# ecpoppenheimer/TensorFlowRayTrace

Measured on AMD Instinct MI355X. Metric: ray-surface intersection tests/sec (fwd+bwd), higher is better.
Workload: dtype f32 ray state, f32 filter + f64 decisions

## Files before the change

### tensorflowraytrace_amd/csrc/tfrt_trace3d.hip

```cpp
#include <vector>

#include <type_traits>
#include "tfrt_common.h"
#include "goal_finish.h"
#include "wave_schedule.h"

namespace tfrt {

constexpr int TILE = 512;
constexpr int KC = 24;

constexpr int ERR_CAPACITY = 1;


__global__ __launch_bounds__(BLOCK) void k_center(const double* __restrict__ fverts, int M,
                                                  double* __restrict__ c0, int32_t* nrays0, int n,
                                                  int32_t* tail8, unsigned int* scan_ticket) {
  if (nrays0 != nullptr) {
    if (threadIdx.x == 0) *nrays0 = n;
    if (threadIdx.x < 8) tail8[threadIdx.x] = 0;
    if (threadIdx.x == 0 && scan_ticket != nullptr) *scan_ticket = 0u;
  }
  __shared__ double red[WAVES][3];
  __shared__ double ctr[3];
// ... 1303 lines not shown
  return __int_as_float(__builtin_amdgcn_readfirstlane(__float_as_int(v)));
}
__device__ __forceinline__ float bcast_f(float v, int src_lane) {
  return __int_as_float(__builtin_amdgcn_readlane(__float_as_int(v), src_lane));
}

template <typename U>
using LdsPtr = __attribute__((address_space(3))) U*;

template <typename RT>
__device__ __forceinline__ void beam_decide(const int nb, const int lane, LdsPtr<const uint32_t> x_pair,
                                         LdsPtr<const RT> rt, LdsPtr<unsigned long long> best_k,
                                         LdsPtr<int32_t> best_i, const double* __restrict__ fverts,
                                         const double eps_int, const double eps_size,
                                         const double eps_start) {
  bool have = false;
  unsigned long long key = 0, old = 0;
  int j = -1;
  const uint32_t xp = lane < nb ? x_pair[lane] : 0u;
  const int slot = (int)(xp & 63u);
  if (lane < nb) {
    double s[3], e[3];
#pragma unroll
    for (int k = 0; k < 3; ++k) {
      s[k] = static_cast<double>(rt[k * 64 + slot]);
      e[k] = static_cast<double>(rt[(3 + k) * 64 + slot]);
    }
    j = (int)(xp >> 6);
    old = best_k[slot];
    double P[9];
    const double* fp = fverts + 9 * (int64_t)j;
#pragma unroll
    for (int k = 0; k < 9; ++k) P[k] = fp[k];
    const TriHit h = exact_triangle<true>(s, e, P, eps_int, eps_size, eps_start);
    if (h.valid) {
      have = true;
      key = dkey(h.ray_u);
    }
  }
  wave_fence();
  if (have) atomicMin((unsigned long long*)&best_k[slot], key);
  wave_fence();
  bool win = false;
  if (have) {
    const unsigned long long now = best_k[slot];
    win = key == now;
    if (win && now < old) best_i[slot] = 0x7FFFFFFF;
  }
  wave_fence();
  if (win) atomicMin((int32_t*)&best_i[slot], j);
  wave_fence();
}

template <typename RT>
struct BeamLds {
  uint16_t slist[BEAM_SLIST];
  uint16_t clist[BEAM_CLIST];
  uint32_t flist[BEAM_FLIST];
  uint32_t x_pair[192];
  float4 ftab[65][4];
  RT rtab[6][64];
  unsigned long long best_k[64];
  int32_t best_i[64];
};

struct BeamScene {
  const float4* susphere;
  const float4* clsphere;
  const float4* csphere;
  const float4* crec;
  const double* fverts;
  const double* c0;
  int n_clusters, n_super;
  double eps_int, eps_size, eps_start;
};

#ifdef TFRT_TICKS
#define TFRT_WI_ARG _wi
#else
#define TFRT_WI_ARG nullptr
#endif

struct BeamCentre {
  double c[3];
  float cf[3];
};
__device__ __forceinline__ BeamCentre beam_centre(const double* __restrict__ c0) {
  BeamCentre o;
#pragma unroll
  for (int k = 0; k < 3; ++k) {
    o.c[k] = c0[k];
    o.cf[k] = uniform_f((float)o.c[k]);
  }
  return o;
}

template <typename T, typename RT>
__device__ __forceinline__ bool beam_pass(BeamLds<RT>& W, const BeamScene& g,
                                          const BeamCentre& ctr, const int lane,
                                          const int bundle, const bool live, const int skip,
                                          const bool first_pass, const int coherent_only,
                                          unsigned* _wi, unsigned* work = nullptr) {
  TFRT_TICK_INIT;
  const float4* __restrict__ susphere = g.susphere;
  const float4* __restrict__ clsphere = g.clsphere;
  const float4* __restrict__ csphere = g.csphere;
  const float4* __restrict__ crec = g.crec;
  const double* __restrict__ fverts = g.fverts;
  const int n_clusters = g.n_clusters, n_super = g.n_super;
  const double eps_int = g.eps_int, eps_size = g.eps_size, eps_start = g.eps_start;
  const float4 never = make_float4(0.f, 0.f, 0.f, -1.f);
  W.best_k[lane] = dkey(INFINITY);
  W.best_i[lane] = -1;
  const double cx = ctr.c[0], cy = ctr.c[1], cz = ctr.c[2];
  const float cxf = ctr.cf[0], cyf = ctr.cf[1], czf = ctr.cf[2];
  auto rel = [](const RT v, const double c, const float cf) -> float {
    if constexpr (sizeof(T) <= 4) return (float)v - cf;
    else return (float)((double)v - c);
  };
  const float es_f = (float)eps_size;
  int xn = 0;

  auto decide = [&](const int nb) {
    TFRT_STAT(28, 1);
    TFRT_WAVE_NOTE(1, 1);
    wave_fence();
    beam_decide<RT>(nb, lane, (LdsPtr<const uint32_t>)&W.x_pair[0],
                    (LdsPtr<const RT>)&W.rtab[0][0], (LdsPtr<unsigned long long>)&W.best_k[0],
                    (LdsPtr<int32_t>)&W.best_i[0], fverts, eps_int, eps_size, eps_start);
  };

  TFRT_STAT(8, 1);
  constexpr int BEAM_ATTEMPTS = 20;
  TFRT_TICK(0);
  float gap = -1.f;
  unsigned long long cuts = 0ull;
  int lo = 0, attempts = 0;
  bool spread = false;
  while (lo < bundle) {
    ++attempts;
    TFRT_STAT(30, 1);
    TFRT_WAVE_NOTE(0, 1);
    const unsigned long long above = lo < 63 ? (cuts >> (lo + 1)) << (lo + 1) : 0ull;
    const int hi = above != 0ull ? __ffsll((long long)above) - 1 : bundle;
    const int len = hi - lo;
    wave_fence();
    RT own[6];
#pragma unroll
    for (int k = 0; k < 6; ++k) own[k] = W.rtab[k][lane];
    const float sx = rel(own[0], cx, cxf), sy = rel(own[1], cy, cyf), sz = rel(own[2], cz, czf);
    const float dx = (float)(own[3] - own[0]), dy = (float)(own[4] - own[1]),
                dz = (float)(own[5] - own[2]);
    const float len2 = dx * dx + dy * dy + dz * dz;
    const bool ok = live && len2 > 0.f && len2 < 3.0e38f;
    const float inv = ok ? __builtin_amdgcn_rsqf(len2) : 0.f;
    const float ux = dx * inv, uy = dy * inv, uz = dz * inv;
    const float rabs = fabsf(sx) + fabsf(sy) + fabsf(sz);
    const bool sel = ok && lane >= lo && lane < hi;
    const float4 su_first = lane < n_super ? susphere[lane] : never;
    const float cnt = (float)__popcll(__ballot(sel));
    bool narrow = true, brute = false;
    int ns = 0, nc = 0, nf = 0;
    Beam bm = {0.f, 0.f, 0.f, 0.f, 0.f, 1.f, 0.f, 0.f, -INFINITY, 1.f, 0.f, 0.f, 0.f, 1.f, 0.f,
               INFINITY, 0.f};
    float ray_t = 0.f, ray_dt = 0.f, ray_terr = 0.f;
    float Ax = 0.f, Ay = 0.f, Mx = 0.f, My = 0.f, Mlen = 0.f, Perr = 0.f, Pm = 0.f;
    if (cnt > 0.f) {
      float swx = sel ? ux : 0.f, swy = sel ? uy : 0.f, swz = sel ? uz : 0.f;
      float sox = sel ? sx : 0.f, soy = sel ? sy : 0.f, soz = sel ? sz : 0.f;
      float Lw = sel ? rabs : 0.f;
      wave_sum4(swx, swy, swz, sox);
      wave_sum2_max(soy, soz, Lw);
      const float wl2 = swx * swx + swy * swy + swz * swz;
      narrow = wl2 > 0.49f * cnt * cnt;
      spread = !narrow;
      const float wi = narrow ? __builtin_amdgcn_rsqf(wl2) : 0.f;
      bm.wx = swx * wi; bm.wy = swy * wi; bm.wz = swz * wi;
      const float icnt = __builtin_amdgcn_rcpf(cnt);
      bm.ox = sox * icnt; bm.oy = soy * icnt; bm.oz = soz * icnt;
      const float cosk = ux * bm.wx + uy * bm.wy + uz * bm.wz;
      if (__any(sel && !(cosk > 0.7f))) narrow = false, spread = true;
      const float px = sx - bm.ox, py = sy - bm.oy, pz = sz - bm.oz;
      const float ts = px * bm.wx + py * bm.wy + pz * bm.wz;
      ray_t = ts;
      ray_dt = dx * bm.wx + dy * bm.wy + dz * bm.wz;
      ray_terr = 1e-5f * (rabs + fabsf(bm.ox) + fabsf(bm.oy) + fabsf(bm.oz));
      {
        const float f0 = fabsf(bm.wx), f1 = fabsf(bm.wy), f2 = fabsf(bm.wz);
        const bool k0 = f0 <= f1 && f0 <= f2, k1 = !k0 && f1 <= f2;
        const float kx = k0 ? 1.f : 0.f, ky = k1 ? 1.f : 0.f, kz = (!k0 && !k1) ? 1.f : 0.f;
        const float cxx = bm.wy * kz - bm.wz * ky, cyy = bm.wz * kx - bm.wx * kz,
                    czz = bm.wx * ky - bm.wy * kx;
// ... 60 lines not shown
      }
      wave_fence();
      TFRT_TICK(2);
      if (narrow && ns > 0) {
        for (int b = 0; b < ns * SUPER; b += 64) {
          const int k = b + lane;
          bool hit = false;
          int cl = 0;
          if (k < ns * SUPER) {
            cl = (int)W.slist[k >> 3] * SUPER + (k & 7);
            if (cl < n_clusters) hit = beam_touch(bm, clsphere[cl]);
          }
          const unsigned long long m = __ballot(hit);
          if (hit) {
            const int pos = nc + rank_below(m);
            if (pos < BEAM_CLIST) W.clist[pos] = (uint16_t)cl;
          }
          nc += __popcll(m);
        }
        narrow = nc <= BEAM_CLIST && n_clusters <= 65536;
      }
      wave_fence();
      TFRT_TICK(3);
      if (narrow && nc > 0) {
        for (int b = 0; b < nc * CLUSTER; b += 64) {
          const int k = b + lane;
          bool hit = false;
          unsigned slot = 0;
          if (k < nc * CLUSTER) {
            slot = (unsigned)W.clist[k >> 4] * CLUSTER + (unsigned)(k & 15);
            hit = beam_touch(bm, csphere[slot]);
          }
          const unsigned long long m = __ballot(hit);
          if (hit) {
            const int pos = nf + rank_below(m);
            if (pos < BEAM_FLIST) W.flist[pos] = slot;
          }
          nf += __popcll(m);
        }
        narrow = nf <= BEAM_FLIST && !(nf > BEAM_WIDE && len > 8 && attempts <= 6);
      }
      wave_fence();
      TFRT_TICK(4);
    }
    if (!narrow) {
      TFRT_TICK(10);
      const bool hopeless = !coherent_only &&
                            ((len == bundle && (spread || (nc > 64 && nc > n_clusters / 4))) ||
                             attempts >= BEAM_ATTEMPTS);
      if (len > 1 && !hopeless) {
        if (cuts == 0ull) {
          const float su = sx * ux + sy * uy + sz * uz;
          const float fx = sx - su * ux, fy = sy - su * uy, fz = sz - su * uz;
          const float gx = fx - __shfl_up(fx, 1, 64), gy = fy - __shfl_up(fy, 1, 64),
                      gz = fz - __shfl_up(fz, 1, 64);
          const float hx = ux - __shfl_up(ux, 1, 64), hy = uy - __shfl_up(uy, 1, 64),
                      hz = uz - __shfl_up(uz, 1, 64);
          const bool prev_ok = __shfl_up(ok ? 1 : 0, 1, 64) != 0;
          gap = 0.f;
          if (ok && prev_ok && lane > 0)
            gap = gx * gx + gy * gy + gz * gz +
                  (sx * sx + sy * sy + sz * sz) * (hx * hx + hy * hy + hz * hz);
          if (!(gap >= 0.f)) gap = 0.f;
        }
        const bool inside = lane > lo && lane < hi;
        const float widest = wave_max_f(inside ? gap : -1.f);
        const unsigned long long at = __ballot(inside && gap == widest);
        const int g = (widest > 0.f && at != 0ull) ? __ffsll((long long)at) - 1 : lo + (len >> 1);
        cuts |= 1ull << g;
        continue;
      }
      if (len == 1 && !hopeless) {
        brute = true;
      } else {
        TFRT_STAT(ns > BEAM_SLIST ? 10 : (nc > BEAM_CLIST ? 11 : (nf > BEAM_FLIST ? 12 : 9)), 1);
        TFRT_STAT(15, lo);
        return false;
      }
    }

    TFRT_STAT(13, nf);
    TFRT_WAVE_NOTE(3, nf);
    TFRT_TICK(5);
    auto reach_now = [&]() {
      const double best = dkey_inv(W.best_k[lane]);
      const float bu = next_up_f((float)best) * ray_dt;
      return ray_t + bu + 1e-5f * fabsf(bu) + ray_terr;
    };
    float myreach = reach_now();
    bool queued = false;
    const int n_cand = brute ? n_clusters * CLUSTER : nf;
    int f0 = 0;
    do {
      const int nb = min(64, n_cand - f0);
      if (work != nullptr) work[1] += (unsigned)nb;
      float4 rec[4] = {never, never, never, never};
      bool touch = false;
      float tnear = INFINITY;
      bool cand = lane < nb;
      if (brute && cand) {
        const float4 sp = csphere[f0 + lane];
        const float vx = sp.x - bm.ox, vy = sp.y - bm.oy, vz = sp.z - bm.oz;
        const float vu = vx * bm.wx + vy * bm.wy + vz * bm.wz;
        const float v2 = vx * vx + vy * vy + vz * vz;
        const float rr = __builtin_amdgcn_sqrtf(sp.w) * 1.000002f + bm.radius(vu, 0.f);
        cand = v2 - vu * vu <= rr * rr + 4e-6f * v2;
      }
      if (cand) {
        const int64_t memb = brute ? (int64_t)(f0 + lane) : (int64_t)W.flist[f0 + lane];
        const float4 r0 = crec[3 * memb], r1 = crec[3 * memb + 1], r2 = crec[3 * memb + 2];
        touch = face_frame(bm, r0, r1, r2, es_f, rec) && __float_as_int(r0.w) >= 0;
        tnear = rec[0].w;
        if (tnear != tnear) tnear = -INFINITY;
        rec[0].w = tnear;
      }
      f0 += 64;
      const bool closing = f0 >= n_cand && hi == bundle;
      const unsigned long long tm = __ballot(touch);
      const int nt = __popcll(tm);
      int place = 0;
      for (unsigned long long rest = tm; rest != 0ull; rest &= rest - 1ull) {
        const int o = __ffsll((long long)rest) - 1;
        const float to = bcast_f(tnear, o);
        place += (to < tnear || (to == tnear && o < lane)) ? 1 : 0;
      }
      wave_fence();
      if (touch) {
        W.ftab[place][0] = rec[0];
        W.ftab[place][1] = rec[1];
        W.ftab[place][2] = rec[2];
        W.ftab[place][3] = rec[3];
      }
      wave_fence();
      TFRT_STAT(27, nt);
      TFRT_TICK(6);
      float span = -INFINITY;
      auto on_face = [&](const float word, int* j, float* thi) {
        const float tn = bcast_f(word, 3);
        *thi = bcast_f(word, 7);
        *j = __float_as_int(bcast_f(word, 14));
        float room, e0, e1, e2;
        face_edges(word, Ax, Ay, Mx, My, Mlen, Perr, Pm, room, e0, e1, e2);
        const bool behind = bm.tmin > -INFINITY && *thi < ray_t - ray_terr;
        return (sel & (*j != skip) & !(myreach < tn) & !behind) &
               (!(e0 > room) & !(e1 > room) & !(e2 > room));
      };
      for (int c = 0;; c += 2) {
        const bool end = c >= nt;
        const bool two = c + 1 < nt;
        const float* recs = reinterpret_cast<const float*>(&W.ftab[end ? 0 : c][0]) + (lane & 15);
        const float word = recs[0], word2 = recs[16];
        const float tn = end ? INFINITY : bcast_f(word, 3);
        const bool flush =
            end ? closing
                : (tn > span && __ballot(sel && !(queued || myreach < INFINITY)) == 0ull);
        while (xn >= 64 || (flush && xn > 0)) {
          const int nd = min(xn, 64);
          wave_fence();
          decide(nd);
          uint32_t tp = 0u, tq = 0u;
          if (lane < xn - nd) tp = W.x_pair[nd + lane];
          if (lane + 64 < xn - nd) tq = W.x_pair[nd + 64 + lane];
          wave_fence();
          if (lane < xn - nd) W.x_pair[lane] = tp;
          if (lane + 64 < xn - nd) W.x_pair[64 + lane] = tq;
          xn -= nd;
          wave_fence();
          if (xn == 0) queued = false;
          myreach = reach_now();
// ... 327 lines not shown
      const double* fp = fnorm + 3 * (int64_t)tri;
#pragma unroll
      for (int q = 0; q < 3; ++q) un[q] = fp[q];
      if (feta != nullptr) {
        const double* fe = feta + 4 * (int64_t)tri;
        n1 = fe[0];
        n2 = fe[1];
        n_in = fe[2];
      } else {
        double n_out;
        face_indices(sc, tri, rid, &n_in, &n_out);
        snell_ratios(n_in, n_out, &n1, &n2);
      }
      const Snell3 f = snell3d_core(s, h, un, n1, n2, n_in == 0.0);
      rec_cls[i] = (uint8_t)(cls | (f.nu > 0.0 ? TAPE_INTERNAL : 0) | (f.reflect ? TAPE_REFLECT : 0));
      double e2[3];
      for (int k = 0; k < 3; ++k) e2[k] = advance(h[k], L, f.w[k]);
      store_ray3(rays_out, stride_out, slot, h, e2);
      ray_id_out[slot] = rid;
      last_tri_out[slot] = tri;
      rec_slot[i] = slot;
      if (prep_next != nullptr) {
        double sr[3], er[3], u[3], scv[3];
        for (int k = 0; k < 3; ++k) {
          sr[k] = static_cast<double>(static_cast<T>(h[k]));
          er[k] = static_cast<double>(static_cast<T>(e2[k]));
        }
        float o[8];
        ray_filter_state(sr, er, c0, o, u, scv);
#pragma unroll
        for (int k = 0; k < 8; ++k) prep_next[k * pstride + slot] = o[k];
      }
    }
  }
  if (!ok) atomicOr(err, ERR_CAPACITY);
}

inline int inplace_bundle(int64_t N) { return N <= 160 * 1024 ? 32 : 64; }
inline size_t inplace_wstride(int64_t N) { return ((size_t)((N > 0 ? N : 1) + 31) / 32 + 63) / 64 * 64; }

template <typename T>
struct InplaceArgs {
  const T* src;
  int64_t src_stride;
  int32_t N, P, bundle, nwaves;
  const InplaceTape* tape;
  const int32_t* sched;
  int32_t ngroups, gshift;
};

#ifndef TFRT_INPLACE_WAVES
#define TFRT_INPLACE_WAVES 5
#endif
#define TFRT_INPLACE_ATTR __attribute__((amdgpu_waves_per_eu(TFRT_INPLACE_WAVES, TFRT_INPLACE_WAVES)))
template <typename T, bool ROWS>
__device__ __forceinline__ void trace_inplace(const InplaceArgs<T>& a, const BeamScene& g) {
  using RT = std::conditional_t<sizeof(T) <= 4, float, double>;
  const int lane = threadIdx.x;
  int qwave = blockIdx.x;
  if (a.sched != nullptr) {
    const int g = __builtin_amdgcn_readfirstlane(a.sched[blockIdx.x >> a.gshift]);
    if ((unsigned)g >= (unsigned)a.ngroups) return;
    qwave = (g << a.gshift) + ((int)blockIdx.x & ((1 << a.gshift) - 1));
    if (qwave >= a.nwaves) return;
  }
  const int q = qwave * a.bundle + lane;
  const bool has = lane < a.bundle && q < a.N;
  const int64_t i = has ? q : 0;
  __shared__ BeamLds<RT> lds;
  BeamLds<RT>& W = lds;
#pragma unroll
  for (int k = 0; k < 6; ++k) W.rtab[k][lane] = static_cast<RT>(a.src[k * a.src_stride + i]);
  bool active = has;
  int skip = -1;
  int p = 0;
  static_assert(sizeof(InplaceTape) % 4 == 0 && sizeof(InplaceTape) / 4 <= 64, "one word per lane");
  const uint32_t tape_words =
      reinterpret_cast<const uint32_t*>(a.tape)[lane < (int)(sizeof(InplaceTape) / 4) ? lane : 0];
  TFRT_WAVE_BEGIN;
  unsigned work[2] = {0u, 0u};
  const BeamCentre centre = beam_centre(g.c0);
  for (; p < a.P; ++p) {
    if (__ballot(active) == 0ull) break;
    beam_pass<T, RT>(W, g, centre, lane, a.bundle, active, skip, p == 0, 1,
                     TFRT_WI_ARG, work);
    wave_fence();
    TFRT_TICK_INIT;
    uint32_t tw = tape_words;
    __asm__ volatile("" : "+v"(tw));
    InplaceTape tq;
    {
      uint32_t w[sizeof(InplaceTape) / 4];
#pragma unroll
      for (int k = 0; k < (int)(sizeof(InplaceTape) / 4); ++k)
        w[k] = (uint32_t)__builtin_amdgcn_readlane((int)tw, k);
      __builtin_memcpy(&tq, w, sizeof(InplaceTape));
    }
    int cls = -1;
    if (active) {
      const int bi = W.best_i[lane];
      const double t = dkey_inv(W.best_k[lane]);
      int cat = 0;
      double un[3] = {0.0, 0.0, 0.0}, fe[3] = {0.0, 0.0, 0.0};
      if (bi >= 0) {
        cat = tq.catagory[bi];
        const double* fp = tq.fnorm + 3 * (int64_t)bi;
#pragma unroll
        for (int k = 0; k < 3; ++k) un[k] = fp[k];
        if (tq.feta != nullptr) {
          const double* fq = tq.feta + 4 * (int64_t)bi;
#pragma unroll
          for (int k = 0; k < 3; ++k) fe[k] = fq[k];
        }
      }
      cls = (bi < 0) ? CLS_DEAD : cat_to_cls(cat);
      const size_t at = (size_t)p * tq.n + i;
      tq.rec_tri[at] = bi;
      tq.rec_t[at] = t;
      int tape = cls;
      if (cls == CLS_ACTIVE) {
        double s[3], e[3], h[3];
#pragma unroll
        for (int k = 0; k < 3; ++k) {
          s[k] = static_cast<double>(W.rtab[k][lane]);
          e[k] = static_cast<double>(W.rtab[3 + k][lane]);
        }
        hit_point(s, e, t, h);
        double n1, n2, n_in;
        if (tq.feta != nullptr) {
          n1 = fe[0];
          n2 = fe[1];
          n_in = fe[2];
        } else {
          n_in = tq.n_table[(int64_t)tq.mat_in[bi] * tq.n_table_stride + i];
          const double n_out = tq.n_table[(int64_t)tq.mat_out[bi] * tq.n_table_stride + i];
          snell_ratios(n_in, n_out, &n1, &n2);
        }
        const Snell3 f = snell3d_core(s, h, un, n1, n2, n_in == 0.0);
        tape |= (f.nu > 0.0 ? TAPE_INTERNAL : 0) | (f.reflect ? TAPE_REFLECT : 0);
        T* out = static_cast<T*>(tq.rays_ws) + (size_t)p * 6 * tq.n;
#pragma unroll
        for (int k = 0; k < 3; ++k) {
          const T hs = static_cast<T>(h[k]);
          const T es = static_cast<T>(advance(h[k], tq.L, f.w[k]));
          out[k * tq.n + i] = hs;
          out[(3 + k) * tq.n + i] = es;
          W.rtab[k][lane] = static_cast<RT>(hs);
          W.rtab[3 + k][lane] = static_cast<RT>(es);
        }
        skip = bi;
      } else {
        active = false;
        if (ROWS) {
          const bool fin = cls == CLS_FINISHED;
          T* fin_rows = static_cast<T*>(tq.fin_rows);
          double h[3] = {0.0, 0.0, 0.0};
          if (fin) {
            double s[3], e[3];
#pragma unroll
            for (int k = 0; k < 3; ++k) {
              s[k] = static_cast<double>(W.rtab[k][lane]);
              e[k] = static_cast<double>(W.rtab[3 + k][lane]);
            }
            hit_point(s, e, t, h);
          }
#pragma unroll
          for (int k = 0; k < 3; ++k) {
            fin_rows[k * tq.fin_cap + i] = fin ? static_cast<T>(W.rtab[k][lane]) : a.src[k * a.src_stride + i];
            fin_rows[(3 + k) * tq.fin_cap + i] = fin ? static_cast<T>(h[k]) : a.src[(3 + k) * a.src_stride + i];
          }
          tq.fin_face[i] = fin ? bi : -1;
          tq.fin_passes[i] = p + 1;
        }
      }
      tq.rec_cls[at] = (uint8_t)tape;
    }
    uint32_t word = 0u;
#pragma unroll
    for (int c = 0; c < 4; ++c) word |= (uint32_t)__popcll(__ballot(cls == c)) << (8 * c);
    if (lane == 0) tq.wcount[(size_t)p * tq.wstride + qwave] = word;
    TFRT_TICK(11);
  }
  InplaceTape te;
  {
    uint32_t w[sizeof(InplaceTape) / 4];
#pragma unroll
    for (int k = 0; k < (int)(sizeof(InplaceTape) / 4); ++k)
      w[k] = (uint32_t)__builtin_amdgcn_readlane((int)tape_words, k);
    __builtin_memcpy(&te, w, sizeof(InplaceTape));
  }
  if (ROWS && active) {
    T* fin_rows = static_cast<T*>(te.fin_rows);
#pragma unroll
    for (int k = 0; k < 6; ++k) fin_rows[k * te.fin_cap + i] = a.src[k * a.src_stride + i];
    te.fin_face[i] = -1;
    te.fin_passes[i] = a.P;
  }
  for (int pp = p + lane; pp < a.P; pp += 64) te.wcount[(size_t)pp * te.wstride + qwave] = 0u;
  if (lane < 2) te.wcount[(size_t)(a.P + lane) * te.wstride + qwave] = work[lane];
  TFRT_WAVE_END(qwave);
}

template <typename T>
__global__ __launch_bounds__(64) TFRT_INPLACE_ATTR void k_trace_inplace(InplaceArgs<T> a, BeamScene g) {
  trace_inplace<T, false>(a, g);
}
template <typename T>
__global__ __launch_bounds__(64) __attribute__((amdgpu_waves_per_eu(4, 4))) void k_trace_inplace_rows(
    InplaceArgs<T> a, BeamScene g) {
  trace_inplace<T, true>(a, g);
}

__global__ __launch_bounds__(1024) void k_inplace_scan(const uint32_t* __restrict__ wcount,
                                                       int nwaves, int wstride, int P, int N, int M,
                                                       int4* __restrict__ wbase,
                                                       int32_t* __restrict__ counts) {
  const int p = blockIdx.x, tid = threadIdx.x, lane = tid & 63, wave = tid >> 6;
  __shared__ int wsum[16][4];
  __shared__ int red[4];
  auto unpack = [](uint32_t w, int v[4]) {
#pragma unroll
    for (int c = 0; c < 4; ++c) v[c] += (int)((w >> (8 * c)) & 0xFFu);
  };
  int before[4] = {0, 0, 0, 0};
  if (p > 0) {
    int acc[4] = {0, 0, 0, 0};
    for (int q = 0; q < p; ++q) {
      const uint32_t* rq = wcount + (size_t)q * wstride;
      for (int k0 = tid; k0 < nwaves; k0 += 8 * 1024) {
        uint32_t w[8];
#pragma unroll
        for (int j = 0; j < 8; ++j) w[j] = (k0 + j * 1024 < nwaves) ? rq[k0 + j * 1024] : 0u;
#pragma unroll
        for (int j = 0; j < 8; ++j) unpack(w[j], acc);
      }
    }
#pragma unroll
    for (int c = 0; c < 4; ++c) {
#pragma unroll
      for (int d = 32; d > 0; d >>= 1) acc[c] += __shfl_xor(acc[c], d, 64);
      if (lane == 0) wsum[wave][c] = acc[c];
    }
    __syncthreads();
    if (tid < 4) {
      int r = 0;
      for (int w = 0; w < 16; ++w) r += wsum[w][tid];
      red[tid] = r;
    }
    __syncthreads();
#pragma unroll
    for (int c = 0; c < 4; ++c) before[c] = red[c];
    __syncthreads();
  }
  const uint4* row4 = reinterpret_cast<const uint4*>(wcount + (size_t)p * wstride);
  int4* out = wbase + (size_t)p * wstride;
  int tot[4] = {0, 0, 0, 0};
  for (int base = 0; base < nwaves; base += 16 * 1024) {
    const int w0 = base + tid * 16;
    uint32_t w[16];
#pragma unroll
    for (int j = 0; j < 4; ++j) {
      const uint4 v = (w0 + 4 * j < nwaves) ? row4[(w0 >> 2) + j] : make_uint4(0u, 0u, 0u, 0u);
      w[4 * j] = v.x;
// ... 269 lines not shown
    typename SweepStore<T>::type* __restrict__ g_out, double* __restrict__ g_src_out,
    int64_t out_stride, double gP[9]);


constexpr int WSUM_SLOTS = 32, WSUM_ROW = 9;
template <int TERMS>
constexpr int wsum_stride(int copies) {
  return WSUM_SLOTS * TERMS * 2 / copies + 2;
}
template <int TERMS>
constexpr int wsum_cells() {
  return 8 * wsum_stride<TERMS>(8);
}
template <int TERMS>
struct WsumCheck {
  static_assert(TERMS == 9 || TERMS == 4, "nine face-vertex terms or the four sums");
  static_assert(4 * wsum_stride<TERMS>(4) <= wsum_cells<TERMS>() &&
                    2 * wsum_stride<TERMS>(2) <= wsum_cells<TERMS>(),
                "wacc holds every tier");
  static_assert(wsum_stride<TERMS>(8) % 4 == 2 && wsum_stride<TERMS>(4) % 4 == 2 &&
                    wsum_stride<TERMS>(2) % 4 == 2,
                "the copies of one cell lie in different LDS banks");
  static_assert(wsum_cells<TERMS>() % 2 == 0, "cleared two cells at a time");
  static constexpr bool ok = true;
};
constexpr int WSUM_CELLS = wsum_cells<9>();
static_assert(WSUM_CELLS == 592 && wsum_cells<4>() == 272 && WsumCheck<9>::ok && WsumCheck<4>::ok,
              "the tiers of wave_face_sums");

template <int TERMS>
__device__ __forceinline__ void wsum_clear(double* wacc) {
  for (int k = 2 * (threadIdx.x & 63); k < wsum_cells<TERMS>(); k += 128)
    *reinterpret_cast<double2*>(wacc + k) = make_double2(0.0, 0.0);
  wave_fence();
}
template <int COPIES, int TERMS>
__device__ __forceinline__ void wsum_fold(double* wacc, const int32_t* wface, int K, int lane,
                                          double* __restrict__ g_fverts) {
  for (int k = lane; k < K; k += 64) {
    double* w = wacc + k;
    double v = w[0];
#pragma unroll
    for (int c = 1; c < COPIES; ++c) v += w[c * wsum_stride<TERMS>(COPIES)];
#pragma unroll
    for (int c = 0; c < COPIES; ++c) w[c * wsum_stride<TERMS>(COPIES)] = 0.0;
    if (v != 0.0) {
      const int f = k / TERMS;
      unsafeAtomicAdd(g_fverts + WSUM_ROW * (int64_t)wface[f] + (k - TERMS * f), v);
    }
  }
}
template <int TERMS>
__device__ __forceinline__ void wave_face_sums(int tri, const double gP[9], double* wacc,
                                               int32_t* wface, double* __restrict__ g_fverts) {
  const int lane = threadIdx.x & 63;
  int slot = -1, ns = 0;
  unsigned long long todo = __ballot(tri >= 0);
  if (todo == 0ull) return;
  while (todo != 0ull && ns < WSUM_SLOTS) {
    const int leader = __ffsll((long long)todo) - 1;
    const int k = __builtin_amdgcn_readlane(tri, leader);
    const bool mine = tri == k;
    if (mine) slot = ns;
    if (lane == leader) wface[ns] = k;
    ++ns;
    todo &= ~__ballot(mine);
  }
  const int copies = ns <= 8 ? 8 : (ns <= 16 ? 4 : 2);
  if (tri >= 0) {
    if (slot >= 0) {
      double* w = &wacc[(lane & (copies - 1)) * wsum_stride<TERMS>(copies) + slot * TERMS];
#pragma unroll
      for (int c = 0; c < TERMS; ++c)
        if (gP[c] != 0.0) unsafeAtomicAdd(w + c, gP[c]);
    } else {
      double* gp = g_fverts + WSUM_ROW * (int64_t)tri;
#pragma unroll
      for (int c = 0; c < TERMS; ++c)
        if (gP[c] != 0.0) unsafeAtomicAdd(gp + c, gP[c]);
    }
  }
  wave_fence();
  if (copies == 8) wsum_fold<8, TERMS>(wacc, wface, ns * TERMS, lane, g_fverts);
  else if (copies == 4) wsum_fold<4, TERMS>(wacc, wface, ns * TERMS, lane, g_fverts);
  else wsum_fold<2, TERMS>(wacc, wface, ns * TERMS, lane, g_fverts);
  wave_fence();
}

template <typename T, int BW>
__global__ __launch_bounds__(64 * BW) void k_backward3d(
    const T* __restrict__ rays_in, int64_t stride_in, const int32_t* __restrict__ n_ptr,
    const int32_t* __restrict__ ray_id_in, const int32_t* __restrict__ rec_tri,
    const double* __restrict__ rec_t, const uint8_t* __restrict__ rec_cls,
    const int32_t* __restrict__ rec_slot, const int32_t* __restrict__ pass_counts,
    tfrt_scene3d sc, double L, double dead_len,
    const typename SweepStore<T>::type* __restrict__ g_child, int64_t child_stride,
    const double* __restrict__ g_fin, int64_t cap_fin, const double* __restrict__ g_act,
    int64_t cap_act, const double* __restrict__ g_stp, int64_t cap_stp,
    const double* __restrict__ g_dead, int64_t cap_dead,
    typename SweepStore<T>::type* __restrict__ g_out, double* __restrict__ g_src_out,
    int64_t out_stride, double* __restrict__ g_fverts,
    typename SweepStore<T>::type* __restrict__ stash_g, int32_t* __restrict__ stash_face,
    int wave_sums) {
  const int n = *n_ptr;
  const int q0 = blockIdx.x * (64 * BW) + threadIdx.x;
  const int i = q0;
  if (wave_sums) {
    if ((q0 & ~63) >= n) return;
    __shared__ __align__(16) double wacc[BW][WSUM_CELLS];
    __shared__ int32_t wface[BW][WSUM_SLOTS];
    const int wave = threadIdx.x >> 6;
    wsum_clear<9>(wacc[wave]);
    double gP[9];
    int tri = -1;
    if (i < n)
      tri = backward_ray<T>(i, rays_in, stride_in, ray_id_in, rec_tri, rec_t, rec_cls, rec_slot,
                            pass_counts, sc, L, dead_len, g_child, child_stride, g_fin, cap_fin,
                            g_act, cap_act, g_stp, cap_stp, g_dead, cap_dead, g_out, g_src_out,
                            out_stride, gP);
    wave_face_sums<9>(tri, gP, wacc[wave], wface[wave], g_fverts);
    return;
  }
  if (i >= n) return;
  double gP[9];
  const int tri = backward_ray<T>(i, rays_in, stride_in, ray_id_in, rec_tri, rec_t, rec_cls,
                                  rec_slot, pass_counts, sc, L, dead_len, g_child, child_stride,
                                  g_fin, cap_fin, g_act, cap_act, g_stp, cap_stp, g_dead, cap_dead,
                                  g_out, g_src_out, out_stride, gP);
  if (stash_face != nullptr) {
    stash_face[i] = tri;
    if (tri >= 0) {
      using S = typename SweepStore<T>::type;
      S* o = stash_g + 9 * (int64_t)i;
#pragma unroll
      for (int c = 0; c < 9; ++c) o[c] = static_cast<S>(gP[c]);
    }
    return;
  }
  if (tri >= 0) {
// ... 468 lines not shown
  const T* src;
  int64_t src_stride;
  const T* rays_ws;
  const int32_t* nrays;
  const int32_t* rec_tri;
  const double* rec_t;
  const uint8_t* rec_cls;
  int64_t n;
  int32_t P;
  double L;
  double* g_src;
  int64_t N;
  double* g_fverts;
  GoalFields gf;
  const double* goal;
  int64_t goal_stride, goal_ray_stride;
  double* partial;
  int32_t* partial_cnt;
  const double* feta;
  const double* face_verts;
  const uint8_t* face_grad_mask;
  const int32_t* sched;
  int32_t ngroups;
  int32_t goal_col[6];
  uint32_t rows_packed;
  int32_t rows_ascending;
};

template <typename T>
static void chain_goal_columns(ChainGoalArgs<T>& g) {
  bool asc = true;
  for (int c = 1; c < g.gf.n; ++c) asc = asc && g.gf.row[c] > g.gf.row[c - 1];
  g.rows_ascending = asc ? 1 : 0;
  g.rows_packed = 0;
  for (int j = 0; j < 6; ++j) g.goal_col[j] = (!asc && j < g.gf.n) ? j : -1;
  for (int c = 0; c < g.gf.n; ++c) {
    g.rows_packed |= (uint32_t)(g.gf.row[c] & 7) << (4 * c);
    if (asc) g.goal_col[g.gf.row[c]] = c;
  }
}

template <typename U>
__device__ __forceinline__ U ld_scalar_base(const U* base, unsigned long long byte_offset) {
  unsigned long long v = reinterpret_cast<unsigned long long>(base);
  __asm__ volatile("" : "+s"(v));
  typedef const U __attribute__((address_space(1))) G;
  return *reinterpret_cast<G*>(v + byte_offset);
}
template <typename U>
__device__ __forceinline__ U ld_lane(const U* base, uint32_t i) {
  return ld_scalar_base(base, (unsigned long long)(i * (uint32_t)sizeof(U)));
}

constexpr int GOAL_ROWS_RUNTIME = -1;
constexpr int GOAL_ROWS_YZ_END = 0b110000;
constexpr __host__ __device__ bool goal_row_set(int rows, int j) { return ((rows >> j) & 1) != 0; }
constexpr __host__ __device__ int goal_row_column(int rows, int j) {
  int c = 0;
  for (int k = 0; k < j; ++k) c += (rows >> k) & 1;
  return c;
}

static int goal_rows_instantiated(const GoalFields& gf) {
  int mask = 0;
  for (int c = 0; c < gf.n; ++c) {
    if (gf.row[c] < 0 || gf.row[c] > 5) return GOAL_ROWS_RUNTIME;
    if (c > 0 && gf.row[c] <= gf.row[c - 1]) return GOAL_ROWS_RUNTIME;
    mask |= 1 << gf.row[c];
  }
  return mask == GOAL_ROWS_YZ_END ? mask : GOAL_ROWS_RUNTIME;
}

template <typename T, bool FIN, bool CHILD, int TERMS, int ROWS>
__device__ __forceinline__ int chain_goal_pass(const ChainGoalArgs<T>& a, int p, int wave, int lane,
                                               int tape, int face, bool fin_lane, double child[6],
                                               double& err, double gP[9]) {
#pragma clang fp contract(off)
  const int cls = tape & 3;
  const size_t off = (size_t)p * a.n;
  const T* rin = p == 0 ? a.src : a.rays_ws + (size_t)(p - 1) * 6 * a.n;
  const int64_t sin = p == 0 ? a.src_stride : a.n;
  const bool child_pass = CHILD && p < a.P - 1;
  const bool fin_here = FIN && fin_lane;
  const bool on_face = face >= 0 && cls != CLS_DEAD;
  const bool with_child = on_face && child_pass && cls == CLS_ACTIVE;
  T ray_w[6];
  double t_rec = 0.0;
  double goal_w[6] = {0, 0, 0, 0, 0, 0};
  uint32_t lv = lane;
  __asm__ volatile("" : "+v"(lv));
  const size_t w0 = (size_t)wave * 64;
#pragma unroll
  for (int k = 0; k < 6; ++k) ray_w[k] = ld_lane(rin + k * sin + w0, lv);
  if (fin_here || on_face) t_rec = ld_lane(a.rec_t + off + w0, lv);
  if (FIN) {
    const int64_t gl = (int64_t)lv * a.goal_ray_stride;
    if constexpr (ROWS != GOAL_ROWS_RUNTIME) {
#pragma unroll
      for (int j = 0; j < 6; ++j) {
        if (goal_row_set(ROWS, j)) {
          const double* gb = a.goal + (int64_t)goal_row_column(ROWS, j) * a.goal_stride +
                             (int64_t)w0 * a.goal_ray_stride;
          if (fin_here) goal_w[j] = ld_scalar_base(gb, (unsigned long long)gl * sizeof(double));
        }
      }
    } else {
// ... 35 lines not shown
    hit_point(s0, e0, t_rec, h0);
#pragma unroll
    for (int k = 0; k < 3; ++k) {
      fin_row[k] = s0[k];
      fin_row[3 + k] = static_cast<double>(static_cast<T>(h0[k]));
    }
    if constexpr (ROWS != GOAL_ROWS_RUNTIME) {
#pragma unroll
      for (int k = 0; k < 6; ++k) {
        if (goal_row_set(ROWS, k)) {
          const double r = fin_row[k] - goal_w[k];
          seed[k] = 2.0 * r;
          err += r * r;
        }
      }
    } else if (a.rows_ascending) {
#pragma unroll
      for (int k = 0; k < 6; ++k) {
        if (a.goal_col[k] >= 0) {
          const double r = fin_row[k] - goal_w[k];
          seed[k] = 2.0 * r;
          err += r * r;
        }
      }
    } else {
#pragma nounroll
      for (int c = 0; c < a.gf.n; ++c) {
        const int row = (a.rows_packed >> (4 * c)) & 7;
        double out_c = 0.0, goal_c = 0.0;
#pragma unroll
        for (int k = 0; k < 6; ++k) {
          if (k == row) out_c = fin_row[k];
          if (k == c) goal_c = goal_w[k];
        }
        const double r = out_c - goal_c;
        const double g = 2.0 * r;
#pragma unroll
        for (int q = 0; q < 6; ++q)
          if (q == row) seed[q] = g;
        err += r * r;
      }
    }
  }
  double gs[3], ge[3];
  const int tri = backward_core_loaded<FIN, CHILD, TERMS>(tape, face, child_pass, s0, e0, Pf, t_rec, n_a,
                                                   n_b, mask_i != 0, a.L, child, seed, gs, ge, gP);
  for (int k = 0; k < 3; ++k) {
    child[k] = gs[k];
    child[3 + k] = ge[k];
  }
  return tri;
}

template <typename T, int TERMS, int ROWS>
__global__ __launch_bounds__(64)
__attribute__((amdgpu_waves_per_eu(TFRT_CHAIN_WAVES, TFRT_CHAIN_WAVES))) void k_backward_chain_goal_inplace(
    ChainGoalArgs<T> a) {
#pragma clang fp contract(off)
  const int n0 = a.nrays[0];
  int wave = blockIdx.x;
  if (a.sched != nullptr) {
    wave = __builtin_amdgcn_readfirstlane(a.sched[blockIdx.x]);
    if ((unsigned)wave >= (unsigned)a.ngroups) return;
  }
  const int i0 = wave * 64 + threadIdx.x;
  const int lane = threadIdx.x;
  if ((i0 & ~63) >= n0) {
    if (lane == 0) {
      a.partial[i0 >> 6] = 0.0;
      if (a.partial_cnt != nullptr) a.partial_cnt[2 * (i0 >> 6)] = a.partial_cnt[2 * (i0 >> 6) + 1] = 0;
    }
    return;
  }
  __builtin_assume(a.feta != nullptr);
  __shared__ __align__(16) double wacc[wsum_cells<TERMS>()];
  __shared__ int32_t wface[WSUM_SLOTS];
  extern __shared__ int2 chain_goal_lds[];
  int2* chain = chain_goal_lds;
  wsum_clear<TERMS>(wacc);
  const int P = a.P;
  int last = -1;
  if (i0 < n0) {
    for (int p = 0; p < P; ++p) {
      const size_t at = (size_t)p * a.n + i0;
      const int tape = a.rec_cls[at], tri = a.rec_tri[at];
      chain[p * 64 + lane] = make_int2(tape, tri);
      last = p;
      if ((tape & 3) != CLS_ACTIVE) break;
    }
  }
  int top = last;
#pragma unroll
  for (int d = 32; d > 0; d >>= 1) top = max(top, __shfl_xor(top, d, 64));
  top = __builtin_amdgcn_readfirstlane(top);
  double child[6] = {0, 0, 0, 0, 0, 0};
  double err = 0.0;
  int n_fin = 0, n_entered = 0;
  for (int p = top; p >= 0; --p) {
    double gP[9];
    int tri = -1;
    const bool here = p <= last;
    int tape = CLS_DEAD, face = -1;
    if (here) {
      const int2 rec = chain[p * 64 + lane];
      tape = rec.x;
      face = max(rec.y, -1);
    }
    const bool fin_here = here && p == last && (tape & 3) == CLS_FINISHED;
    const unsigned long long fin_m = __ballot(fin_here);
    const bool fin_role = here && fin_m != 0ull && !(p < P - 1 && (tape & 3) == CLS_ACTIVE);
    if (fin_role)
      tri = chain_goal_pass<T, true, false, TERMS, ROWS>(a, p, wave, lane, tape, face, fin_here, child, err, gP);
    if (here && !fin_role)
      tri = chain_goal_pass<T, false, true, TERMS, ROWS>(a, p, wave, lane, tape, face, false, child, err, gP);
    n_fin += __popcll(fin_m);
    n_entered += __popcll(__ballot(here));
    wave_face_sums<TERMS>(tri, gP, wacc, wface, a.g_fverts);
  }
  if (a.g_src != nullptr && i0 < n0) {
    for (int k = 0; k < 6; ++k) a.g_src[k * a.N + i0] = child[k];
  }
#pragma unroll
  for (int d = 32; d > 0; d >>= 1) err += __shfl_xor(err, d, 64);
  if (lane == 0) {
    a.partial[i0 >> 6] = err;
    if (a.partial_cnt != nullptr) {
      a.partial_cnt[2 * (i0 >> 6)] = n_fin;
      a.partial_cnt[2 * (i0 >> 6) + 1] = n_entered;
    }
  }
}


template <typename T>
__global__ __launch_bounds__(BLOCK) void k_finalize_seam(
    const T* __restrict__ rays, int64_t stride, int n, int chunks,
    const double* __restrict__ part_t, const int32_t* __restrict__ part_i, int64_t part_stride,
    const double* __restrict__ fverts, int M, double eps_int, double eps_size, double eps_start,
    double* x, double* y, double* z, uint8_t* valid, double* ray_u, double* trig_u,
    double* trig_v, int32_t* gather_trig) {
  const int i = blockIdx.x * BLOCK + threadIdx.x;
  if (i >= n) return;
  double bt = INFINITY;
  int bi = -1;
  for (int c = 0; c < chunks; ++c) {
    const double t = part_t[c * part_stride + i];
    if (t < bt) {
      bt = t;
      bi = part_i[c * part_stride + i];
    }
  }
  const int tri = bi < 0 ? 0 : bi;
  double s[3], e[3], P[9], h[3] = {0, 0, 0};
  TriHit th;
  th.ray_u = th.trig_u = th.trig_v = 0.0;
  th.valid = false;
  if (M > 0) {
    load_ray3(rays, stride, i, s, e);
    for (int q = 0; q < 9; ++q) P[q] = fverts[9 * (int64_t)tri + q];
    th = exact_triangle(s, e, P, eps_int, eps_size, eps_start);
    hit_point(s, e, th.ray_u, h);
  }
  x[i] = h[0];
  y[i] = h[1];
  z[i] = h[2];
  valid[i] = bi >= 0;
  ray_u[i] = bi >= 0 ? th.ray_u : INFINITY;
  trig_u[i] = th.trig_u;
  trig_v[i] = th.trig_v;
  gather_trig[i] = tri;
}


struct Plan3 {
  int R, ray_blocks, chunks, chunk_faces, nblk;
  int g_blocks, g_chunks, g_chunk_clusters;
};

struct Accel3 {
  const int32_t* order;
  int n_clusters;
// ... 1015 lines not shown
```

Measured before the change: 142700 billion.

## Raise f32 in-place trace occupancy with smaller candidate chunks and rematerialized lanes

The f32 in-place trace kernel now targets 6 waves per EU instead of 5 and walks candidates in chunks of 32, which also shrinks the LDS face table. Lane indices and ray indices are recomputed late, with asm barriers that stop the compiler from holding them in registers across the pass. The chain-goal backward kernel gets a separate waves-per-EU knob and rematerializes its lane index the same way, using bpermute-based shuffles. The aim is lower register pressure and higher occupancy, at the cost of twice as many chunk iterations and some risk of spills.

```diff
diff --git a/tensorflowraytrace_amd/csrc/tfrt_trace3d.hip b/tensorflowraytrace_amd/csrc/tfrt_trace3d.hip
--- a/tensorflowraytrace_amd/csrc/tfrt_trace3d.hip
+++ b/tensorflowraytrace_amd/csrc/tfrt_trace3d.hip
@@ -1379,13 +1379,13 @@
   wave_fence();
 }
 
-template <typename RT>
+template <typename RT, int CHUNK = 64>
 struct BeamLds {
   uint16_t slist[BEAM_SLIST];
   uint16_t clist[BEAM_CLIST];
   uint32_t flist[BEAM_FLIST];
   uint32_t x_pair[192];
-  float4 ftab[65][4];
+  float4 ftab[CHUNK + 1][4];
   RT rtab[6][64];
   unsigned long long best_k[64];
   int32_t best_i[64];
@@ -1422,9 +1422,9 @@
   return o;
 }
 
-template <typename T, typename RT>
-__device__ __forceinline__ bool beam_pass(BeamLds<RT>& W, const BeamScene& g,
-                                          const BeamCentre& ctr, const int lane,
+template <typename T, typename RT, int CHUNK = 64>
+__device__ __forceinline__ bool beam_pass(BeamLds<RT, CHUNK>& W, const BeamScene& g,
+                                          const BeamCentre& ctr, const int lane_in,
                                           const int bundle, const bool live, const int skip,
                                           const bool first_pass, const int coherent_only,
                                           unsigned* _wi, unsigned* work = nullptr) {
@@ -1437,7 +1437,15 @@
   const int n_clusters = g.n_clusters, n_super = g.n_super;
   const double eps_int = g.eps_int, eps_size = g.eps_size, eps_start = g.eps_start;
   const float4 never = make_float4(0.f, 0.f, 0.f, -1.f);
-  W.best_k[lane] = dkey(INFINITY);
+  constexpr bool LATE = CHUNK < 64;
+  int lane = lane_in;
+  unsigned long long no_hit = dkey(INFINITY);
+  if constexpr (LATE) {
+    uint32_t top = (uint32_t)(no_hit >> 32);
+    __asm__ volatile("" : "+s"(top));
+    no_hit = ((unsigned long long)top << 32) | (uint32_t)no_hit;
+  }
+  W.best_k[lane] = no_hit;
   W.best_i[lane] = -1;
   const double cx = ctr.c[0], cy = ctr.c[1], cz = ctr.c[2];
   const float cxf = ctr.cf[0], cyf = ctr.cf[1], czf = ctr.cf[2];
@@ -1465,6 +1473,7 @@
   int lo = 0, attempts = 0;
   bool spread = false;
   while (lo < bundle) {
+    if constexpr (LATE) __asm__ volatile("" : "+v"(lane));
     ++attempts;
     TFRT_STAT(30, 1);
     TFRT_WAVE_NOTE(0, 1);
@@ -1631,11 +1640,20 @@
         if (cuts == 0ull) {
           const float su = sx * ux + sy * uy + sz * uz;
           const float fx = sx - su * ux, fy = sy - su * uy, fz = sz - su * uz;
-          const float gx = fx - __shfl_up(fx, 1, 64), gy = fy - __shfl_up(fy, 1, 64),
-                      gz = fz - __shfl_up(fz, 1, 64);
-          const float hx = ux - __shfl_up(ux, 1, 64), hy = uy - __shfl_up(uy, 1, 64),
-                      hz = uz - __shfl_up(uz, 1, 64);
-          const bool prev_ok = __shfl_up(ok ? 1 : 0, 1, 64) != 0;
+          auto up1 = [&](const float v) -> float {
+            if constexpr (LATE)
+              return __int_as_float(
+                  __builtin_amdgcn_ds_bpermute((lane - (lane > 0 ? 1 : 0)) << 2, __float_as_int(v)));
+            else
+              return __shfl_up(v, 1, 64);
+          };
+          const float gx = fx - up1(fx), gy = fy - up1(fy), gz = fz - up1(fz);
+          const float hx = ux - up1(ux), hy = uy - up1(uy), hz = uz - up1(uz);
+          bool prev_ok;
+          if constexpr (LATE)
+            prev_ok = __builtin_amdgcn_ds_bpermute((lane - (lane > 0 ? 1 : 0)) << 2, ok ? 1 : 0) != 0;
+          else
+            prev_ok = __shfl_up(ok ? 1 : 0, 1, 64) != 0;
           gap = 0.f;
           if (ok && prev_ok && lane > 0)
             gap = gx * gx + gy * gy + gz * gz +
@@ -1671,7 +1689,7 @@
     const int n_cand = brute ? n_clusters * CLUSTER : nf;
     int f0 = 0;
     do {
-      const int nb = min(64, n_cand - f0);
+      const int nb = min(CHUNK, n_cand - f0);
       if (work != nullptr) work[1] += (unsigned)nb;
       float4 rec[4] = {never, never, never, never};
       bool touch = false;
@@ -1693,7 +1711,7 @@
         if (tnear != tnear) tnear = -INFINITY;
         rec[0].w = tnear;
       }
-      f0 += 64;
+      f0 += CHUNK;
       const bool closing = f0 >= n_cand && hi == bundle;
       const unsigned long long tm = __ballot(touch);
       const int nt = __popcll(tm);
@@ -2127,11 +2145,21 @@
 #ifndef TFRT_INPLACE_WAVES
 #define TFRT_INPLACE_WAVES 5
 #endif
-#define TFRT_INPLACE_ATTR __attribute__((amdgpu_waves_per_eu(TFRT_INPLACE_WAVES, TFRT_INPLACE_WAVES)))
-template <typename T, bool ROWS>
+#ifndef TFRT_INPLACE_F32_WAVES
+#define TFRT_INPLACE_F32_WAVES 6
+#endif
+template <typename T>
+constexpr int inplace_waves() {
+  return std::is_same<T, float>::value ? TFRT_INPLACE_F32_WAVES : TFRT_INPLACE_WAVES;
+}
+template <typename T>
+constexpr int inplace_chunk() {
+  return std::is_same<T, float>::value && TFRT_INPLACE_F32_WAVES > 5 ? 32 : 64;
+}
+template <typename T, bool ROWS, int CHUNK>
 __device__ __forceinline__ void trace_inplace(const InplaceArgs<T>& a, const BeamScene& g) {
   using RT = std::conditional_t<sizeof(T) <= 4, float, double>;
-  const int lane = threadIdx.x;
+  int lane = threadIdx.x;
   int qwave = blockIdx.x;
   if (a.sched != nullptr) {
     const int g = __builtin_amdgcn_readfirstlane(a.sched[blockIdx.x >> a.gshift]);
@@ -2139,14 +2167,19 @@
     qwave = (g << a.gshift) + ((int)blockIdx.x & ((1 << a.gshift) - 1));
     if (qwave >= a.nwaves) return;
   }
-  const int q = qwave * a.bundle + lane;
-  const bool has = lane < a.bundle && q < a.N;
-  const int64_t i = has ? q : 0;
-  __shared__ BeamLds<RT> lds;
-  BeamLds<RT>& W = lds;
-#pragma unroll
-  for (int k = 0; k < 6; ++k) W.rtab[k][lane] = static_cast<RT>(a.src[k * a.src_stride + i]);
-  bool active = has;
+  auto ray_index = [&](bool* has) -> int64_t {
+    const int q = qwave * a.bundle + lane;
+    *has = lane < a.bundle && q < a.N;
+    return *has ? q : 0;
+  };
+  __shared__ BeamLds<RT, CHUNK> lds;
+  BeamLds<RT, CHUNK>& W = lds;
+  bool active;
+  {
+    const int64_t i = ray_index(&active);
+#pragma unroll
+    for (int k = 0; k < 6; ++k) W.rtab[k][lane] = static_cast<RT>(a.src[k * a.src_stride + i]);
+  }
   int skip = -1;
   int p = 0;
   static_assert(sizeof(InplaceTape) % 4 == 0 && sizeof(InplaceTape) / 4 <= 64, "one word per lane");
@@ -2157,8 +2190,10 @@
   const BeamCentre centre = beam_centre(g.c0);
   for (; p < a.P; ++p) {
     if (__ballot(active) == 0ull) break;
-    beam_pass<T, RT>(W, g, centre, lane, a.bundle, active, skip, p == 0, 1,
-                     TFRT_WI_ARG, work);
+    __asm__ volatile("" : "+v"(lane));
+    beam_pass<T, RT, CHUNK>(W, g, centre, lane, a.bundle, active, skip, p == 0, 1,
+                            TFRT_WI_ARG, work);
+    __asm__ volatile("" : "+v"(lane));
     wave_fence();
     TFRT_TICK_INIT;
     uint32_t tw = tape_words;
@@ -2173,6 +2208,8 @@
     }
     int cls = -1;
     if (active) {
+      bool has;
+      const int64_t i = ray_index(&has);
       const int bi = W.best_i[lane];
       const double t = dkey_inv(W.best_k[lane]);
       int cat = 0;
@@ -2265,6 +2302,8 @@
     __builtin_memcpy(&te, w, sizeof(InplaceTape));
   }
   if (ROWS && active) {
+    bool has;
+    const int64_t i = ray_index(&has);
     T* fin_rows = static_cast<T*>(te.fin_rows);
 #pragma unroll
     for (int k = 0; k < 6; ++k) fin_rows[k * te.fin_cap + i] = a.src[k * a.src_stride + i];
@@ -2277,13 +2316,15 @@
 }
 
 template <typename T>
-__global__ __launch_bounds__(64) TFRT_INPLACE_ATTR void k_trace_inplace(InplaceArgs<T> a, BeamScene g) {
-  trace_inplace<T, false>(a, g);
+__global__ __launch_bounds__(64)
+__attribute__((amdgpu_waves_per_eu(inplace_waves<T>(), inplace_waves<T>()))) void k_trace_inplace(
+    InplaceArgs<T> a, BeamScene g) {
+  trace_inplace<T, false, inplace_chunk<T>()>(a, g);
 }
 template <typename T>
 __global__ __launch_bounds__(64) __attribute__((amdgpu_waves_per_eu(4, 4))) void k_trace_inplace_rows(
     InplaceArgs<T> a, BeamScene g) {
-  trace_inplace<T, true>(a, g);
+  trace_inplace<T, true, 64>(a, g);
 }
 
 __global__ __launch_bounds__(1024) void k_inplace_scan(const uint32_t* __restrict__ wcount,
@@ -2659,8 +2700,8 @@
 }
 template <int TERMS>
 __device__ __forceinline__ void wave_face_sums(int tri, const double gP[9], double* wacc,
-                                               int32_t* wface, double* __restrict__ g_fverts) {
-  const int lane = threadIdx.x & 63;
+                                               int32_t* wface, double* __restrict__ g_fverts,
+                                               int lane) {
   int slot = -1, ns = 0;
   unsigned long long todo = __ballot(tri >= 0);
   if (todo == 0ull) return;
@@ -2692,6 +2733,11 @@
   else if (copies == 4) wsum_fold<4, TERMS>(wacc, wface, ns * TERMS, lane, g_fverts);
   else wsum_fold<2, TERMS>(wacc, wface, ns * TERMS, lane, g_fverts);
   wave_fence();
+}
+template <int TERMS>
+__device__ __forceinline__ void wave_face_sums(int tri, const double gP[9], double* wacc,
+                                               int32_t* wface, double* __restrict__ g_fverts) {
+  wave_face_sums<TERMS>(tri, gP, wacc, wface, g_fverts, (int)(threadIdx.x & 63));
 }
 
 template <typename T, int BW>
@@ -3266,6 +3312,13 @@
   return ld_scalar_base(base, (unsigned long long)(i * (uint32_t)sizeof(U)));
 }
 
+__device__ __forceinline__ double shfl_xor_lane(double v, int d, uint32_t lane) {
+  const int at = (int)((lane ^ (uint32_t)d) << 2);
+  const int lo = __builtin_amdgcn_ds_bpermute(at, __double2loint(v));
+  const int hi = __builtin_amdgcn_ds_bpermute(at, __double2hiint(v));
+  return __hiloint2double(hi, lo);
+}
+
 constexpr int GOAL_ROWS_RUNTIME = -1;
 constexpr int GOAL_ROWS_YZ_END = 0b110000;
 constexpr __host__ __device__ bool goal_row_set(int rows, int j) { return ((rows >> j) & 1) != 0; }
@@ -3407,9 +3460,16 @@
   return tri;
 }
 
+#ifndef TFRT_CHAIN_GOAL_WAVES
+#define TFRT_CHAIN_GOAL_WAVES 5
+#endif
+constexpr int chain_goal_waves(int terms, int rows) {
+  return terms == 4 && rows != GOAL_ROWS_RUNTIME ? TFRT_CHAIN_GOAL_WAVES : TFRT_CHAIN_WAVES;
+}
 template <typename T, int TERMS, int ROWS>
 __global__ __launch_bounds__(64)
-__attribute__((amdgpu_waves_per_eu(TFRT_CHAIN_WAVES, TFRT_CHAIN_WAVES))) void k_backward_chain_goal_inplace(
+__attribute__((amdgpu_waves_per_eu(chain_goal_waves(TERMS, ROWS), chain_goal_waves(TERMS, ROWS))))
+void k_backward_chain_goal_inplace(
     ChainGoalArgs<T> a) {
 #pragma clang fp contract(off)
   const int n0 = a.nrays[0];
@@ -3456,8 +3516,10 @@
     int tri = -1;
     const bool here = p <= last;
     int tape = CLS_DEAD, face = -1;
+    uint32_t lp = lane;
+    __asm__ volatile("" : "+v"(lp));
     if (here) {
-      const int2 rec = chain[p * 64 + lane];
+      const int2 rec = chain[p * 64 + lp];
       tape = rec.x;
       face = max(rec.y, -1);
     }
@@ -3470,18 +3532,21 @@
       tri = chain_goal_pass<T, false, true, TERMS, ROWS>(a, p, wave, lane, tape, face, false, child, err, gP);
     n_fin += __popcll(fin_m);
     n_entered += __popcll(__ballot(here));
-    wave_face_sums<TERMS>(tri, gP, wacc, wface, a.g_fverts);
-  }
-  if (a.g_src != nullptr && i0 < n0) {
-    for (int k = 0; k < 6; ++k) a.g_src[k * a.N + i0] = child[k];
-  }
-#pragma unroll
-  for (int d = 32; d > 0; d >>= 1) err += __shfl_xor(err, d, 64);
-  if (lane == 0) {
-    a.partial[i0 >> 6] = err;
+    wave_face_sums<TERMS>(tri, gP, wacc, wface, a.g_fverts, (int)lp);
+  }
+  uint32_t lv = lane;
+  __asm__ volatile("" : "+v"(lv));
+  const int i1 = wave * 64 + (int)lv;
+  if (a.g_src != nullptr && i1 < n0) {
+    for (int k = 0; k < 6; ++k) a.g_src[k * a.N + i1] = child[k];
+  }
+#pragma unroll
+  for (int d = 32; d > 0; d >>= 1) err += shfl_xor_lane(err, d, lv);
+  if (lv == 0) {
+    a.partial[wave] = err;
     if (a.partial_cnt != nullptr) {
-      a.partial_cnt[2 * (i0 >> 6)] = n_fin;
-      a.partial_cnt[2 * (i0 >> 6) + 1] = n_entered;
+      a.partial_cnt[2 * wave] = n_fin;
+      a.partial_cnt[2 * wave + 1] = n_entered;
     }
   }
 }
```

Result: faster. 152100 billion (median of 6 runs) (+6.6%).
